# lorenzsp/EMRI_FrequencyDomainWaveforms

Hardware: AMD Instinct MI355X
Metric: FD waveforms/sec (2 yr, dt=10 s, ~3000 modes) at 1/2/4/8 GPUs; mode-sum HBM GB/s (higher is better)
Workload: dtype f64

## Files before the change

emri_frequencydomainwaveforms_amd/_lib.py:

```python

import ctypes
import os

_HERE = os.path.dirname(os.path.abspath(__file__))
LIB_PATH = os.environ.get("EFD_LIB") or os.path.join(_HERE, "libemrifd.so")

EFD_OK = 0
EFD_ERR_ARG = -1
EFD_ERR_HIP = -2
EFD_ERR_WORKSPACE = -3
EFD_CAUSTIC_SPA = 0
EFD_CAUSTIC_UNIFORM = 1
EFD_LOGLIKE_SCRATCH = 1024
EFD_INNER_SCRATCH = 2048
EFD_FISHER_MAX_PARAMS = 16
EFD_FISHER_SCRATCH = 139264
EFD_OVERLAP_MAX_ROWS = 64
EFD_OVERLAP_SCRATCH = 197632
EFD_BATCH_MAX = 16
EFD_HANN_ROWS_MAX = 16
EFD_HANN_LOCAL_PARTIALS = 4096
EFD_TD_SPLIT_SCRATCH = 1024
EFD_PAIR_MAX_ROWS = 64
EFD_PAIR_SCRATCH = 655360
EFD_DH_MAX_ROWS = 64
EFD_DH_SCRATCH = 196608
EFD_WINDOW_MAX_ROWS = 16
EFD_MODES_AMP_OVERFLOW = 1
EFD_TRAJ_MAX_LEN = 1024
EFD_NOISE_MAX_ROWS = 16
EFD_NOISE_DRAWS_PER_LAUNCH = 256
EFD_NOISE_SCRATCH = 1048576
EFD_TRAJ_OK = 0
EFD_TRAJ_BAD_SOURCE = 1
EFD_TRAJ_TOO_LONG = 2
EFD_TRAJ_STEP_FAILED = 3
EFD_TRAJ_STEP_CAP = 4
EFD_TRAJ_NO_BRACKET = 5

EXPORTED_SYMBOLS = (
    "efd_version",
    "efd_build_id",
# ... 35 lines not shown
    "efd_hann_loglike",
    "efd_hann_loglike_local",
    "efd_hann_loglike_local_partials",
    "efd_cosw_polarizations",
    "efd_cosw_loglike",
    "efd_loglike",
    "efd_inner_product",
    "efd_fisher_gram",
    "efd_overlap_rows",
    "efd_pair_stats",
    "efd_td_split_pair_stats",
    "efd_dh_hh_rows",
    "efd_window_rows",
    "efd_modesum_cpu",
    "efd_modesum_cpu_stats",
    "efd_spline_build_cpu",
    "efd_polarizations_cpu",
    "efd_loglike_cpu",
    "efd_inner_product_cpu",
    "efd_fisher_gram_cpu",
    "efd_overlap_rows_cpu",
    "efd_td_split_cpu",
    "efd_td_split_loglike_cpu",
    "efd_pair_stats_cpu",
    "efd_td_split_pair_stats_cpu",
    "efd_dh_hh_rows_cpu",
    "efd_window_rows_cpu",
    "efd_cpu_threads",
    "efd_cpu_last_error",
    "efd_host_trajectory",
# ... 286 lines not shown
    for name in ("efd_td_split_pair_stats", "efd_td_split_pair_stats_cpu"):
        getattr(lib, name).restype = ctypes.c_int
        getattr(lib, name).argtypes = [vp, i64, i64, i32, dbl, vp, i64, vp, vp, vp, vp, vp]
    for name in ("efd_dh_hh_rows", "efd_dh_hh_rows_cpu"):
        getattr(lib, name).restype = ctypes.c_int
        getattr(lib, name).argtypes = [vp, i64, i32, vp, vp, i32, i64, vp, vp, vp]
    for name in ("efd_window_rows", "efd_window_rows_cpu"):
        getattr(lib, name).restype = ctypes.c_int
        getattr(lib, name).argtypes = [vp, i64, ctypes.POINTER(vp), i32, vp, i64, vp]
    if hasattr(lib, "efd_modesum_cpu"):
        lib.efd_modesum_cpu.restype = ctypes.c_int
        lib.efd_modesum_cpu.argtypes = [ctypes.POINTER(ModesumArgs), vp, sz, vp]
        lib.efd_modesum_cpu_stats.restype = ctypes.c_int
        lib.efd_modesum_cpu_stats.argtypes = [ctypes.POINTER(i64), ctypes.POINTER(i64),
                                              ctypes.POINTER(i32)]
        lib.efd_spline_build_cpu.restype = ctypes.c_int
        lib.efd_spline_build_cpu.argtypes = [vp, ctypes.c_int, vp, ctypes.c_int, vp, vp]
        lib.efd_polarizations_cpu.restype = ctypes.c_int
        lib.efd_polarizations_cpu.argtypes = [vp, i64, i64, vp, vp, vp]
        lib.efd_loglike_cpu.restype = ctypes.c_int
        lib.efd_loglike_cpu.argtypes = [vp, vp, vp, i32, i64, vp, vp, vp]
        lib.efd_inner_product_cpu.restype = ctypes.c_int
        lib.efd_inner_product_cpu.argtypes = [vp, vp, vp, i32, i64, vp, vp, vp]
        lib.efd_fisher_gram_cpu.restype = ctypes.c_int
        lib.efd_fisher_gram_cpu.argtypes = [vp, i64, i32, i32, vp, vp, i64, vp, vp, vp, vp]
        lib.efd_cpu_threads.restype = ctypes.c_int
        lib.efd_cpu_threads.argtypes = [ctypes.c_int]
        lib.efd_cpu_last_error.restype = ctypes.c_int
        lib.efd_cpu_last_error.argtypes = [ctypes.c_char_p, ctypes.c_int]
    if hasattr(lib, "efd_host_trajectory"):
# ... 75 lines not shown
```

emri_frequencydomainwaveforms_amd/cputwin.py:

```python

import ctypes

import numpy as np

from . import _lib

CAUSTIC = {"spa": _lib.EFD_CAUSTIC_SPA, "uniform": _lib.EFD_CAUSTIC_UNIFORM}


def _lib_cpu():
    lib = _lib.load()
    if not hasattr(lib, "efd_modesum_cpu"):
        raise _lib.EFDError("libemrifd.so lacks efd_modesum_cpu: rebuild it")
    return lib


def set_threads(n):
    return int(_lib_cpu().efd_cpu_threads(int(n)))


def last_error():
    buf = ctypes.create_string_buffer(512)
    _lib_cpu().efd_cpu_last_error(buf, 512)
    return buf.value.decode(errors="replace")


def modesum(t, amp, phi_phi, phi_r, f_phi, f_r, m, n, ylm_p, ylm_m, freq, scale=1.0 + 0.0j,
            caustic="uniform", grid_symmetric=None, out=None, polarizations=False, k0=0,
            accumulate=False):
    lib = _lib_cpu()
    f64 = lambda x: np.ascontiguousarray(x, dtype=np.float64)
    c128 = lambda x: np.ascontiguousarray(x, dtype=np.complex128)
    i32 = lambda x: np.ascontiguousarray(x, dtype=np.int32)
    t, phi_phi, phi_r, f_phi, f_r, freq = (f64(x) for x in (t, phi_phi, phi_r, f_phi, f_r, freq))
    amp, ylm_p, ylm_m = c128(amp), c128(ylm_p), c128(ylm_m)
    m, n = i32(m), i32(n)
    nt, K = amp.shape
    nf = len(freq)
    if grid_symmetric is None:
        grid_symmetric = bool(np.array_equal(freq, -freq[::-1]))
    hp = hc = None
    new = np.zeros if accumulate else np.empty
    if polarizations:
        hp = new(nf - k0, dtype=np.complex128)
        hc = new(nf - k0, dtype=np.complex128)
        S = None
    else:
        S = out if out is not None else new(nf, dtype=np.complex128)
    p = lambda x: x.ctypes.data if x is not None else None
    sc = complex(scale)
    a = _lib.ModesumArgs(
        t=p(t), phi_phi=p(phi_phi), phi_r=p(phi_r), f_phi=p(f_phi), f_r=p(f_r), nt=nt,
        amp=p(amp), m=p(m), n=p(n), ylm_p=p(ylm_p), ylm_m=p(ylm_m), K=K, freq=p(freq), nf=nf,
        grid_symmetric=1 if grid_symmetric else 0, scale_re=sc.real, scale_im=sc.imag,
        caustic=CAUSTIC[caustic], accumulate=1 if accumulate else 0, out=p(S),
        prof_begin=None, prof_end=None, hp=p(hp), hc=p(hc), k0=int(k0))
    rc = lib.efd_modesum_cpu(ctypes.byref(a), None, 0, None)
    if rc != _lib.EFD_OK:
        raise _lib.EFDError(f"efd_modesum_cpu failed ({rc}): {last_error()}")
    return (hp, hc) if polarizations else S


def stats():
    c, e, g = ctypes.c_int64(0), ctypes.c_int64(0), ctypes.c_int32(0)
    _lib_cpu().efd_modesum_cpu_stats(ctypes.byref(c), ctypes.byref(e), ctypes.byref(g))
    return int(c.value), int(e.value), int(g.value)


def loglike(h, d, w):
    lib = _lib_cpu()
    h = np.ascontiguousarray(h, dtype=np.complex128)
    d = np.ascontiguousarray(d, dtype=np.complex128)
    w = np.ascontiguousarray(w, dtype=np.float64)
    if h.shape != d.shape or w.shape != d.shape or d.ndim != 2:
        raise ValueError("loglike: h, d, w must share one [nchan][nbin] shape")
# ... 7 lines not shown
```

emri_frequencydomainwaveforms_amd/csrc/emrifd.hip:

```cpp

#include "emrifd_layout.h"

#define EFD_VERSION 100

static thread_local std::string g_err;

int efdhip::fail(int code, const std::string& msg) {
    g_err = msg;
    return code;
}

namespace {

constexpr int NWAVE = TILE / 64;
constexpr int XCD_GROUP = 1024 / TILE;
constexpr int SEGWIN = TILE;
constexpr int PIECES = (int)sizeof(Item) / 16;
constexpr int B_PIECE = (int)offsetof(Item, b) / 16;
constexpr int ROUNDS = 2;
constexpr int NC = (ROUNDS * TILE) / PIECES;


__device__ __forceinline__ bool seg_hits_tile(int2 lh, int32_t tlo, int32_t thi) {
    return lh.y > tlo && lh.x < thi;
// ... 274 lines not shown
    r.shift = fdneg ? -192 : 192;
    r.kth = fdneg ? -KTH0 / VS : KTH0 / VS;
    return r;
}
__device__ __forceinline__ uint64_t class_mask(double x, int32_t cls) {
    uint64_t m;
    asm volatile("v_cmp_class_f64_e64 %0, %1, %2" : "=s"(m) : "v"(x), "s"(cls));
    return m;
}
__device__ __forceinline__ double ftz_select(bool ok, double v) {
    return __hiloint2double(ok ? __double2hiint(v) : 0, __double2loint(v));
}
constexpr int HDR_HB = TILE_LANES < 1024 ? 10 : 11;
constexpr uint32_t HDR_HM = (1u << HDR_HB) - 1u;
constexpr int HDR_S = 2 * HDR_HB, HDR_J = 2 * HDR_HB + 1, HDR_FD = 2 * HDR_HB + 4;
static_assert(FAST_J < 8, "header: jser in 3 bits");
static_assert(TILE_LANES < 2048 && HDR_FD + 2 <= 32, "header: one 32-bit word");
__device__ __forceinline__ uint32_t hdr_pack(uint32_t lo, uint32_t hi, int s, int32_t jser,
                                             int32_t fdneg) {
    return lo | (hi << HDR_HB) | ((uint32_t)s << HDR_S) | ((uint32_t)jser << HDR_J) |
           ((uint32_t)fdneg << HDR_FD);
}
__device__ __forceinline__ int32_t hdr_lo(uint32_t ha) { return (int32_t)(ha & HDR_HM); }
__device__ __forceinline__ int32_t hdr_hi(uint32_t ha) {
    return (int32_t)((ha >> HDR_HB) & HDR_HM);
}
__device__ __forceinline__ int hdr_s(uint32_t ha) { return (int)((ha >> HDR_S) & 1u); }
__device__ __forceinline__ uint32_t hdr_jser(uint32_t ha) { return (ha >> HDR_J) & 7u; }
__device__ __forceinline__ uint32_t hdr_fdneg(uint32_t ha) { return (ha >> HDR_FD) & 3u; }
__device__ __forceinline__ uint32_t hdr_safe(uint32_t ha) { return (ha >> (HDR_FD + 1)) & 1u; }
__device__ __forceinline__ bool hdr_test(uint32_t ha, uint32_t mask) {
    asm volatile("" : "+s"(ha));
    return (ha & mask) != 0;
}
__device__ __forceinline__ bool hdr_j3(uint32_t ha) {
    asm volatile("" : "+s"(ha));
    return hdr_jser(ha) >= 3u;
}
__device__ __forceinline__ bool hdr_j4(uint32_t ha) {
    asm volatile("" : "+s"(ha));
    return hdr_jser(ha) >= 4u;
}
__device__ __forceinline__ void spa_simple(const Item* __restrict__ it, double sfk, double stfk,
                                           const double2* __restrict__ sct, const RecSign& rs,
                                           double& wr, double& wi, double& w) {
    const double u = sfk - it->gx;
    const double tt = fma(fma(fma(it->ic[0], u, it->ic[1]), u, it->ic[2]), u, it->ic[3]);
    w = tt - it->tj;
    const double ph = fma(fma(fma(it->ph[0], w, it->ph[1]), w, it->ph[2]), w, it->ph[3]);
    const double fd = fma(fma(it->fd[0], w, it->fd[1]), w, it->fd[2]);
    const double amp = rsqrt_pos_sum(fabs(fd));
    const double psi0 = fma(stfk, tt, -ph);
    const double fdds = fma(fma(it->fdd[0], w, it->fdd[1]), w, it->fdd[2]);
    const double a3 = amp * amp * amp;
    const double t3 = fdds * a3;
    const double ww = t3 * t3;
// ... 13 lines not shown
    const double amp = rsqrt_pos_sum(fabs(fd));
    const double psi0 = fma(stfk, tt, -ph);
    const double fdds = fma(fma(it->fdd[0], w, it->fdd[1]), w, it->fdd[2]);
    const double a3 = amp * amp * amp;
    const double t3 = fdds * a3;
    const double ww = t3 * t3;
    const double uu = ww * ww;
    const double r = fma(45.7, uu * uu, 1.0 - uu);
    const double thn = ww * fma(-14.733333333333333333, uu, 1.0);
    const double am = amp * r;
    double sn, cs;
    sincos_tab(psi0, rs.shift, sct, sn, cs, thn, true, rs.kth, COS_A);
    wr = am * cs;
    wi = am * sn;
}
template <bool MASK, int NB>
__device__ __forceinline__ void env_record(const Item* __restrict__ it, const double* fk,
                                           const double* tfk, const double2* __restrict__ sct,
                                           const RecSign& rs, const uint64_t* am, double* wr,
                                           double* wi, double* w) {
    const double* e = env_of(it);
#pragma unroll
    for (int i = 0; i < NB; ++i) {
        const double u = fk[i] - it->gx;
        const double tt = fma(fma(fma(it->ic[0], u, it->ic[1]), u, it->ic[2]), u, it->ic[3]);
        w[i] = tt - it->tj;
        const double ph = fma(fma(fma(it->ph[0], w[i], it->ph[1]), w[i], it->ph[2]), w[i], it->ph[3]);
        const double psi0 = fma(tfk[i], tt, -ph);
        double amp = e[0];
#pragma unroll
        for (int c = 1; c <= ENV_DEG; ++c) amp = fma(amp, w[i], e[c]);
        if (MASK) amp = ftz_select(__builtin_amdgcn_inverse_ballot_w64(am[i]), amp);
        sincos_tab_amp(psi0, rs.shift, sct, amp, wr[i], wi[i]);
    }
}
template <int CAUSTIC>
__device__ __forceinline__ void spa_fast_m(const Item* __restrict__ it, double sfk, double stfk,
                                           uint32_t ha, uint64_t actm,
                                           const double2* __restrict__ sct,
                                           const RecSign& rs, double& wr, double& wi, double& w,
                                           uint64_t& needm) {
    const double u = sfk - it->gx;
    const double tt = fma(fma(fma(it->ic[0], u, it->ic[1]), u, it->ic[2]), u, it->ic[3]);
    w = tt - it->tj;
    const double ph = fma(fma(fma(it->ph[0], w, it->ph[1]), w, it->ph[2]), w, it->ph[3]);
    const double fd = fma(fma(it->fd[0], w, it->fd[1]), w, it->fd[2]);
    const double afd = fabs(fd);
    uint64_t goodm = ~0ull;
// ... 63 lines not shown
    exp_add(ay >= 153.0 ? 8 : ay >= 75.0 ? 9 : ay >= 48.0 ? 10 : ay >= 29.4 ? 11
            : ay >= 23.1 ? 12 : ay >= 20.3 ? 13 : ay >= 18.4 ? 14 : 15);
}
__device__ __forceinline__ void exp_chunk_balance(const int* wv) {
    int mx = 0, sm = 0;
    for (int w = 0; w < NWAVE; ++w) { mx = max(mx, wv[w]); sm += wv[w]; }
    exp_add(24, (unsigned long long)mx);
    exp_add(25, (unsigned long long)sm);
    exp_add(26);
}
__device__ __forceinline__ void exp_record(int64_t tile) {
    exp_add(0);
    if (tile < 16384) atomicAdd(&g_exp_tile[tile], 1u);
}
__device__ __forceinline__ void exp_record_class(uint32_t ha, bool partial) {
    exp_add(31 + min((int)hdr_jser(ha), 4));
    if (hdr_safe(ha)) exp_add(29);
    if (partial) exp_add(37);
    if (hdr_jser(ha) >= 3u) exp_add(38);
    if (!hdr_safe(ha)) exp_add(39);
}
template <int NB>
__device__ __forceinline__ void exp_cold(const bool (&need)[NB], int lane) {
    unsigned long long nl = 0;
#pragma unroll
    for (int i = 0; i < NB; ++i) nl += __popcll(__ballot(need[i]));
    if (lane == 0) {
        exp_add(16);
        exp_add(17, nl);
    }
}
__device__ __forceinline__ void exp_tile_clock(int64_t tile, unsigned long long t_start) {
    if (tile < 16384)
        g_exp_tclk[tile] = ((t_start & 0xffffffffull) << 32) |
// ... 308 lines not shown
        __syncthreads();

        for (int c = 0; c < nchunk; ++c) {
            tid = opq(tid0);
            lane = tid & 63;
            if (c + 1 < nchunk) EFD_GLDS(c + 1, (c + 1) & 1);
            const int nin = (int)rfl((uint32_t)min(NC, cnt - c * NC));
            const Item* stg = stage[c & 1];
            uint32_t hdr = 0;
            if (lane < nin) {
                const uint32_t kl = keys[c * NC + lane];
                const int sl = (int)(kl & 1);
                const Item* il = stg + lane;
                const uint32_t lo = (uint32_t)min(max(il->klo[sl] - tlo, 0), TILE_LANES);
                const uint32_t hi = (uint32_t)min(max(il->khi[sl] - tlo, 0), TILE_LANES);
                hdr = hdr_pack(lo, hi, sl, il->jser, il->fdneg);
            }
            EFD_EXP_DO(int nev = 0; if (c > 0 && tid == 0) exp_chunk_balance(wimb[(c - 1) & 1]);)
            for (int ii = 0; ii < nin; ++ii) {
                const uint32_t ha = (uint32_t)__builtin_amdgcn_readlane((int)hdr, ii);
                const int s = hdr_s(ha);
                const int32_t klo = tlo + hdr_lo(ha);
                const int32_t khi = tlo + hdr_hi(ha);
                const Item* it = stg + ii;
                if (khi <= e_lo || klo >= e_hi) {
                    EFD_EXP_DO(if (lane == 0) exp_add(3);)
                    continue;
                }
                EFD_EXP_DO(++nev; if (lane == 0) exp_record(tile);)
                bool anyneed = false;
                bool need[NB];
// ... 4 lines not shown
                        for (int i = 0; i < NB; ++i) {
                            fk[i] = -fk[i];
                            tfk[i] = -tfk[i];
                            own_i[i] = -own_i[i];
                            mir_i[i] = -mir_i[i];
                        }
                        s_cur = s;
                    }
                    const int J = CAUSTIC == EFD_CAUSTIC_UNIFORM ? (int)hdr_jser(ha) : FAST_J;
                    const double* xo = &it->b[0][0][0];
                    const double* xm = &it->b[1][0][0];
                    double wr[NB], wi[NB], w[NB];
                    uint64_t needm[NB], needany = 0;
                    const RecSign rs = rec_sign(hdr_fdneg(ha));
                    EFD_EXP_DO(if (lane == 0) exp_record_class(ha, e_lo < klo || khi < e_hi);)
                    if (CAUSTIC == EFD_CAUSTIC_UNIFORM && !hdr_test(ha, 7u << HDR_J)) {
                        if (!hdr_test((uint32_t)((e_lo - klo) | (khi - e_hi)) >> 31, 1u)) {
                            env_record<false, NB>(it, fk, tfk, sctab, rs, nullptr, wr, wi, w);
                        } else {
                            uint64_t am[NB];
#pragma unroll
                            for (int i = 0; i < NB; ++i) {
                                const int32_t base = e_lo + 64 * i;
                                am[i] = lane_range_mask(klo - base, khi - base);
                            }
                            env_record<true, NB>(it, fk, tfk, sctab, rs, am, wr, wi, w);
                        }
#pragma unroll
                        for (int i = 0; i < NB; ++i) need[i] = false;
                    } else
                    if (CAUSTIC == EFD_CAUSTIC_UNIFORM &&
                        !hdr_test(((uint32_t)((e_lo - klo) | (khi - e_hi)) >> 31) |
                                  ((hdr_jser(ha) + 5u) >> 3) |
                                  (hdr_safe(ha) ^ 1u), 1u)) {
#pragma unroll
                        for (int i = 0; i < NB; ++i) {
                            spa_simple(it, fk[i], tfk[i], sctab, rs, wr[i], wi[i], w[i]);
                            need[i] = false;
                        }
                    } else
                    if (CAUSTIC == EFD_CAUSTIC_UNIFORM &&
// ... 1404 lines not shown
```

emri_frequencydomainwaveforms_amd/csrc/emrifd_cpu.cpp:

```cpp
#include <algorithm>
#include <cmath>
#include <cstdint>
#include <cstdio>
#include <cstdlib>
#include <cstring>
#include <numeric>
#include <string>
#include <vector>

#include <omp.h>

#include "../../include/emrifd.h"
#include "emrifd_cpu_internal.h"

namespace efdcpu {

struct double2 {
    double x, y;
};
#define EFD_TABLE static const
#include "spa_tables.inc"
#undef EFD_TABLE

#include "emrifd_constants.h"
// ... 292 lines not shown
                    if (G0 != 0.0) {
                        const double xv = -(2.0 * G1) / (6.0 * G0);
                        if (xv > 0.0 && xv < dt) gmax = std::fmax(gmax, std::fabs(qv(3.0 * G0, 2.0 * G1, G2, xv)));
                    }
                    const double ymin = gmax > 0.0 ? TWO_PI * fdmin * fdmin * fdmin / (3.0 * gmax * gmax) / 1.1
                                                   : INFINITY;
                    int J = FAST_J;
                    for (int jj = 1; jj < FAST_J; ++jj)
                        if (ymin >= JSER_Y[jj]) { J = jj; break; }
                    it.jser = J;
                    it.envc = 0;
                    if (env_on && ymin >= ENV_MIN_Y) {
                        const double gq[3] = {3.0 * G0, 2.0 * G1, G2};
                        EnvFit E;
                        if (env_fit(it.fd, gq, it.dtj, (it.fdneg & 1) != 0, E)) {
                            it.envc = 1;
                            for (int c = 0; c <= ENV_DEG; ++c) it.env[c] = E.a[c];
                            for (int c = 0; c < 4; ++c) it.phE[c] = it.ph[c] - E.th[c];
                        }
                    }
                    const double Fj = knotF(a->f_phi, a->f_r, m, n, j);
                    const double Fj1 = knotF(a->f_phi, a->f_r, m, n, j + 1);
                    const double xlo = sg > 0 ? Fj : Fj1, xhi = sg > 0 ? Fj1 : Fj;
                    const bool strict = sg > 0 ? (j == ra) : (j + 1 == rb);
                    auto upper = [&](double v) { return (int64_t)(std::upper_bound(freq, freq + nf, v) - freq); };
                    auto lower = [&](double v) { return (int64_t)(std::lower_bound(freq, freq + nf, v) - freq); };
                    int64_t lo0 = upper(-xhi);
                    int64_t hi0 = strict ? lower(-xlo) : upper(-xlo);
                    int64_t lo1 = strict ? upper(xlo) : lower(xlo);
                    int64_t hi1 = lower(xhi);
                    auto clampr = [](int64_t& lo, int64_t& hi, int64_t lim) {
                        if (lo > lim) lo = lim;
// ... 200 lines not shown
        const int64_t qi = (int64_t)q;
        const int off = (int)((qi + shift) & 511);
        const double ts = T.s[off], tc = T.c[off];
        const double z = r * r;
        const double sr = std::fma(r * z, -1.6666666666666666e-01, r);
        const double cr = std::fma(z, COS_B, c0);
        const double sn = std::fma(ts, cr, tc * sr);
        const double cs = std::fma(tc, cr, -ts * sr);
        wr[i] = am * cs;
        wi[i] = am * sn;
        wv[i] = w;
        need[i] = !good;
    }
}

void spa_fast_env(const Rec& it, int s, const double* fk, int n, double* wr, double* wi,
                  double* wv, unsigned char* need) {
    const SinCosTable& T = sctab();
    const double sgn = s ? 1.0 : -1.0;
    const int shift = (it.fdneg & 1) ? -192 : 192;
    constexpr double INV_STEP = 81.48733086305042;
    constexpr double STEP_1 = 0.01227184630308513;
    constexpr double SHIFTER = 6755399441055744.0;
#pragma omp simd
    for (int i = 0; i < n; ++i) {
        const double g = sgn * fk[i];
        const double u = g - it.gx;
        const double tt = std::fma(std::fma(std::fma(it.ic[0], u, it.ic[1]), u, it.ic[2]), u, it.ic[3]);
        const double w = tt - it.tj;
        const bool good = (w >= 0.0) & (w < it.dtj);
        const double ph = std::fma(std::fma(std::fma(it.phE[0], w, it.phE[1]), w, it.phE[2]), w, it.phE[3]);
        const double psi0 = std::fma(TWO_PI * g, tt, -ph);
        double A = it.env[0];
        for (int c = 1; c <= ENV_DEG; ++c) A = std::fma(A, w, it.env[c]);
        const double am = good ? A : 0.0;
        const double qs = std::fma(psi0, INV_STEP, SHIFTER);
        const double q = qs - SHIFTER;
        const double r = std::fma(-q, STEP_1, psi0);
        const int64_t qi = (int64_t)q;
        const int off = (int)((qi + shift) & 511);
        const double ts = T.s[off], tc = T.c[off];
        const double z = r * r;
        const double sr = std::fma(r * z, -1.6666666666666666e-01, r);
        const double cr = std::fma(z, COS_B, COS_A);
        const double sn = std::fma(ts, cr, tc * sr);
        const double cs = std::fma(tc, cr, -ts * sr);
        wr[i] = am * cs;
        wi[i] = am * sn;
        wv[i] = w;
// ... 16 lines not shown
            for (int64_t t = it.klo[s] / TL; t <= (it.khi[s] - 1) / TL; ++t) ++cnt[t];
        }
    L.off.assign(ntiles + 1, 0);
    for (int64_t t = 0; t < ntiles; ++t) L.off[t + 1] = L.off[t] + cnt[t];
    L.ent.resize(L.off[ntiles]);
    std::vector<int64_t> pos(L.off.begin(), L.off.end() - 1);
    for (size_t r = 0; r < nrec; ++r)
        for (int s = 0; s < 2; ++s) {
            const Rec& it = P.recs[r];
            if (it.khi[s] <= it.klo[s]) continue;
            for (int64_t t = it.klo[s] / TL; t <= (it.khi[s] - 1) / TL; ++t)
                L.ent[pos[t]++] = (uint32_t)((r << 1) | (size_t)s);
        }
}

int modesum(const efd_modesum_args* a) {
    if (!a) return fail(EFD_ERR_ARG, "efd_modesum_cpu: NULL argument");
    if (!a->t || !a->phi_phi || !a->phi_r || !a->f_phi || !a->f_r || !a->amp || !a->m || !a->n ||
        !a->ylm_p || !a->ylm_m || !a->freq)
        return fail(EFD_ERR_ARG, "efd_modesum_cpu: NULL array");
    const bool pol = a->hp != nullptr || a->hc != nullptr;
    if (pol && (!a->hp || !a->hc || !a->grid_symmetric || a->k0 < 0 || a->k0 > a->nf))
        return fail(EFD_ERR_ARG, "efd_modesum_cpu: hp/hc need both pointers, a symmetric grid and 0 <= k0 <= nf");
    if (!a->out && !pol) return fail(EFD_ERR_ARG, "efd_modesum_cpu: no output (out or hp/hc)");
    if (a->nt < 2 || a->nt > MAX_NT) return fail(EFD_ERR_ARG, "efd_modesum_cpu: nt out of range");
    if (a->K <= 0 || a->K > MAX_K) return fail(EFD_ERR_ARG, "efd_modesum_cpu: K out of range [1, 8192]");
    if (a->nf <= 0 || a->nf >= (int64_t)INT32_MAX) return fail(EFD_ERR_ARG, "efd_modesum_cpu: nf out of range");
    if (a->caustic != EFD_CAUSTIC_SPA && a->caustic != EFD_CAUSTIC_UNIFORM)
        return fail(EFD_ERR_ARG, "efd_modesum_cpu: unknown caustic mode");
    for (int i = 1; i < a->nt; ++i)
        if (!(a->t[i] > a->t[i - 1])) return fail(EFD_ERR_ARG, "efd_modesum_cpu: t not increasing");
    const bool paired = a->grid_symmetric != 0;
    const int64_t nf = a->nf;
    const int64_t nl = paired ? (nf + 1) / 2 : nf;
    const int64_t nl1 = paired ? ((nf % 2) ? nl - 1 : nl) : nf;
    Prep P;
    const int rc = prepare(a, P, paired, nl, nl1);
    if (rc != EFD_OK) return rc;
    g_stats[0] = P.contributions;
    g_stats[1] = P.evaluations;
    g_stats[2] = P.G;
    const int64_t ntiles = (nl + TL - 1) / TL;
    TileLists L;
    build_tile_lists(P, ntiles, L);
    const double* freq = a->freq;
    const int caustic = a->caustic;
    const bool acc = a->accumulate != 0;
    const int64_t k0 = a->k0;
#pragma omp parallel num_threads(nthreads())
    {
        alignas(64) double fk[TL], own_r[TL], own_i[TL], mir_r[TL], mir_i[TL];
        alignas(64) double wr[TL], wi[TL], wv[TL];
// ... 4 lines not shown
            const int nln = (int)std::min<int64_t>(TL, nl - tlo);
            for (int i = 0; i < nln; ++i) fk[i] = freq[tlo + i];
            std::fill(own_r, own_r + TL, 0.0);
            std::fill(own_i, own_i + TL, 0.0);
            std::fill(mir_r, mir_r + TL, 0.0);
            std::fill(mir_i, mir_i + TL, 0.0);
            for (int64_t e = L.off[tile]; e < L.off[tile + 1]; ++e) {
                const uint32_t key = L.ent[e];
                const Rec& it = P.recs[key >> 1];
                const int s = (int)(key & 1u);
                const int lo = (int)std::max<int64_t>(it.klo[s] - tlo, 0);
                const int hi = (int)std::min<int64_t>(it.khi[s] - tlo, nln);
                if (hi <= lo) continue;
                const int n = hi - lo;
                if (caustic == EFD_CAUSTIC_UNIFORM) {
                    if (it.envc) spa_fast_env(it, s, fk + lo, n, wr, wi, wv, need);
                    else if (it.jser >= 3) spa_fast<EFD_CAUSTIC_UNIFORM, true>(it, s, fk + lo, n, wr, wi, wv, need);
                    else spa_fast<EFD_CAUSTIC_UNIFORM, false>(it, s, fk + lo, n, wr, wi, wv, need);
                } else {
                    spa_fast<EFD_CAUSTIC_SPA, false>(it, s, fk + lo, n, wr, wi, wv, need);
                }
                const double* X = &it.b[s][0][0];
                const double* Z = &it.b[1 - s][0][0];
                const double so = s ? -1.0 : 1.0;
#pragma omp simd
                for (int i = 0; i < n; ++i) {
                    const double w = wv[i];
                    const double xr = cubic(X, w), xi = cubic(X + 4, w);
                    const double zr = cubic(Z, w), zi = cubic(Z + 4, w);
                    const int k = lo + i;
                    own_r[k] = std::fma(-xi, wi[i], std::fma(xr, wr[i], own_r[k]));
// ... 68 lines not shown
    std::snprintf(buf, (size_t)len, "%s", efdcpu::g_err.c_str());
    return EFD_OK;
}

int efd_modesum_cpu(const efd_modesum_args* a, void* workspace, size_t workspace_bytes,
                    void* stream) {
    (void)workspace; (void)workspace_bytes; (void)stream;
    return efdcpu::modesum(a);
}

int efd_modesum_cpu_stats(int64_t* contributions, int64_t* evaluations, int32_t* groups) {
    if (contributions) *contributions = efdcpu::g_stats[0];
    if (evaluations) *evaluations = efdcpu::g_stats[1];
    if (groups) *groups = (int32_t)efdcpu::g_stats[2];
    return EFD_OK;
}

int efd_spline_build_cpu(const double* x, int n, const double* y, int ninterp, double* coef,
                         void* stream) {
    (void)stream;
    if (!x || !y || !coef || n < 2 || ninterp <= 0 || n > efdcpu::MAX_NT)
        return efdcpu::fail(EFD_ERR_ARG, "efd_spline_build_cpu: bad arguments");
    for (int i = 1; i < n; ++i)
        if (!(x[i] > x[i - 1])) return efdcpu::fail(EFD_ERR_ARG, "efd_spline_build_cpu: x not increasing");
#pragma omp parallel num_threads(efdcpu::nthreads())
    {
        std::vector<double> cp, dp, s, tq((size_t)(n - 1) * 4);
#pragma omp for schedule(static)
        for (int q = 0; q < ninterp; ++q) {
            efdcpu::spline_nak(n, [&](int i) { return x[i]; },
// ... 11 lines not shown
```

emri_frequencydomainwaveforms_amd/csrc/emrifd_prepare.hip:

```cpp

#include "emrifd_layout.h"

namespace {

constexpr int SPLINE_PF = 8;

__device__ __forceinline__ double spl_rcp(double x) {
#ifdef EFD_EXP_EXACT_RCP
    return 1.0 / x;
#endif
    double y = __builtin_amdgcn_rcp(x);
    double e = fma(-x, y, 1.0);
    y = fma(y, e, y);
    e = fma(-x, y, 1.0);
    return fma(y, e, y);
}

template <class FX, class FY, class FCP, class FDP, class FOUT>
__device__ void spline_not_a_knot(int n, FX X, FY Y, FCP CP, FDP DP, FOUT OUT) {
    if (n < 2) return;
    if (n == 2) {
        const double dx = X(1) - X(0);
        const double slope = (Y(1) - Y(0)) / dx;
        OUT(0, 0, 0.0); OUT(0, 1, 0.0); OUT(0, 2, slope); OUT(0, 3, Y(0));
// ... 1178 lines not shown
    if ((threadIdx.x & 63) == 0) {
        red[0][threadIdx.x >> 6] = contrib;
        red[1][threadIdx.x >> 6] = ev;
        red[2][threadIdx.x >> 6] = eev;
    }
    __syncthreads();
    if (threadIdx.x == 0) {
        const unsigned long long c = red[0][0] + red[0][1] + red[0][2] + red[0][3];
        const unsigned long long e = red[1][0] + red[1][1] + red[1][2] + red[1][3];
        const unsigned long long x = red[2][0] + red[2][1] + red[2][2] + red[2][3];
        if (c) atomicAdd((unsigned long long*)&hdr->contributions, c);
        if (e) atomicAdd((unsigned long long*)&hdr->evaluations, e);
        if (x) atomicAdd((unsigned long long*)&hdr->env_evaluations, x);
    }
}
__global__ __launch_bounds__(256) void k_items(const PrepBatch B) {
    const PrepView V(B);
    items_body(V.t, V.f_phi, V.f_r, V.gm, V.gn, V.gstart, V.nt, V.K, V.coefA, V.coefT, V.runs,
               V.freq, V.nf, V.paired, V.nl, V.nl1, V.items, V.ranges, V.header,
               (V.pcr & 1) != 0, V.env != 0);
}

__device__ __forceinline__ void slot_segment(const PrepView& V, int i,
                                             const int4* __restrict__ ranges, int G, int2& lh,
                                             int4& info) {
    const int h = i / (2 * MAXRUNS), r = (i >> 1) % MAXRUNS, sb = i & 1;
    const int ni = V.nt - 1;
    lh = make_int2(0, 0);
    info = make_int4(0, 0, 0, 0);
    const int32_t* rr = V.runs + (size_t)h * 4 * MAXRUNS + 4 * r;
    if (h < G && rr[2] != 0) {
// ... 508 lines not shown
```

emri_frequencydomainwaveforms_amd/csrc/env_fit.inc:

```

constexpr int ENV_DEG = 6;
constexpr double ENV_TOL_A = 1e-11;
constexpr double ENV_TOL_T = 1e-10;
constexpr double ENV_MIN_Y = 153.0;

struct EnvFit {
    double a[ENV_DEG + 1];
    double th[4];
};

EFD_HD inline void env_exact(const double* fd, const double* g, double thsign, double w, double& A,
                             double& th) {
    const double fdv = fma(fma(fd[0], w, fd[1]), w, fd[2]);
    const double fddv = fma(fma(g[0], w, g[1]), w, g[2]);
    const double r = env_rsqrt(fabs(fdv));
    const double r2 = r * r;
    const double wv = (3.0 / TWO_PI) * (fddv * fddv) * (r2 * r2 * r2);
    const double u = wv * wv;
    const double rho = fma(fma(fma(KRH[3], u, KRH[2]), u, KRH[1]), u, KRH[0]);
    const double thn = wv * fma(fma(fma(KTHN[3], u, KTHN[2]), u, KTHN[1]), u, KTHN[0]);
    A = rho * r;
    th = thsign * thn;
}

// ... 20 lines not shown
     -585.14285714285714286, 527.19549756118696301, -364.83060405905322015,
     130.20653506929482857}};
constexpr double ENV_W3[4][7] = {
    {-0.10165443621355265414, 0.10702091160166934744, 0.11930124891586627315,
     -0.14285714285714285714, -0.18986684997799971916, 0.30584819351622459786,
     0.90220807501493501199},
    {2.5185918758768087888, -2.2932605173801433673, -3.3408618646193829832,
     2.2857142857142857143, 6.1911009588307362656, 1.2760219621512775191,
     -6.6373067005735819373},
    {-8.6629029186417365166, 6.4590248426552300049, 11.945320391387904255,
     -2.2857142857142857143, -14.795559485599257537, -5.4417862874263641567,
     12.781617743338509665},
    {7.1481735539934153939, -3.9669370433605313872, -8.9136266256623872642, 0.0,
     8.9136266256623872642, 3.9669370433605313872, -7.1481735539934153939}};

template <int R>
EFD_HD inline void env_apply(const double (*M)[7], const double* f, double dtj, double* out) {
    const double r = 1.0 / dtj;
    double rk = 1.0;
#pragma unroll
    for (int i = 0; i < R; ++i) {
        double p = M[i][0] * f[0];
#pragma unroll
        for (int k = 1; k < 7; ++k) p = fma(M[i][k], f[k], p);
        out[R - 1 - i] = p * rk;
        rk *= r;
    }
}

EFD_HD inline bool env_fit(const double* fd, const double* g, double dtj, bool fdneg, EnvFit& E) {
    constexpr double X7[7] = {0.97492791218182360702, 0.78183148246802980871,
                              0.43388373911755812048, 0.0, -0.43388373911755812048,
                              -0.78183148246802980871, -0.97492791218182360702};
    constexpr double SC[8] = {0.0, 0.049515566048790436882, 0.18825509907063323474,
                              0.38873953302184279786, 0.61126046697815720214,
                              0.81174490092936676526, 0.95048443395120956312, 1.0};
    const double thsign = fdneg ? -KTH0 : KTH0;
    double fa[7], ft[7];
#pragma unroll
    for (int k = 0; k < 7; ++k) env_exact(fd, g, thsign, dtj * fma(0.5, X7[k], 0.5), fa[k], ft[k]);
    env_apply<ENV_DEG + 1>(ENV_W7, fa, dtj, E.a);
    env_apply<4>(ENV_W3, ft, dtj, E.th);
    double amax = 0.0, ea = 0.0, et = 0.0;
#pragma unroll
    for (int k = 0; k < 8; ++k) {
        const double w = dtj * SC[k];
        double A, th;
        env_exact(fd, g, thsign, w, A, th);
        double pa = E.a[0];
        for (int i = 1; i <= ENV_DEG; ++i) pa = fma(pa, w, E.a[i]);
        const double pt = fma(fma(fma(E.th[0], w, E.th[1]), w, E.th[2]), w, E.th[3]);
        amax = fmax(amax, fabs(A));
        ea = fmax(ea, fabs(pa - A));
        et = fmax(et, fabs(pt - th));
        if (!(fabs(A) < INFINITY && fabs(pa) < INFINITY && fabs(pt) < INFINITY)) return false;
    }
    return ea <= ENV_TOL_A * amax && et <= ENV_TOL_T;
}
```

include/emrifd.h:

```cpp
#ifndef EMRIFD_H
#define EMRIFD_H

#include <stddef.h>
#include <stdint.h>

#ifdef __cplusplus
extern "C" {
#endif

#define EFD_OK 0
#define EFD_ERR_ARG (-1)
#define EFD_ERR_HIP (-2)
#define EFD_ERR_WORKSPACE (-3)

#define EFD_CAUSTIC_SPA 0
#define EFD_CAUSTIC_UNIFORM 1

int efd_version(void);

const char* efd_build_id(void);

int efd_last_error(char* buf, int len);

int efd_spline_build(const double* x, int n, const double* y, int ninterp, double* coef,
// ... 176 lines not shown
                            const uint8_t* keep, double* out, double* scratch, void* stream);

#define EFD_DH_MAX_ROWS 64
#define EFD_DH_SCRATCH 196608
int efd_dh_hh_rows(const double* h, int64_t row_stride, int32_t nrow, const double* d,
                   const double* w, int32_t nchan, int64_t nbin, double* out, double* scratch,
                   void* stream);

#define EFD_WINDOW_MAX_ROWS 16
int efd_window_rows(const double* h, int64_t n, const double* const* win, int32_t nwin,
                    double* out, int64_t out_stride, void* stream);

int efd_modesum_cpu(const efd_modesum_args* a, void* workspace, size_t workspace_bytes,
                    void* stream);
int efd_modesum_cpu_stats(int64_t* contributions, int64_t* evaluations, int32_t* groups);
int efd_spline_build_cpu(const double* x, int n, const double* y, int ninterp, double* coef,
                         void* stream);
int efd_polarizations_cpu(const double* S, int64_t nf, int64_t k0, double* hp, double* hc,
                          void* stream);
int efd_loglike_cpu(const double* h, const double* d, const double* w, int32_t nchan,
                    int64_t nbin, double* out, double* scratch, void* stream);
int efd_inner_product_cpu(const double* a, const double* b, const double* w, int32_t nchan,
                          int64_t nbin, double* out, double* scratch, void* stream);
int efd_fisher_gram_cpu(const double* h, int64_t row_stride, int32_t nparam, int32_t npoint,
                        const double* coef, const double* w, int64_t nelem, double* dh,
                        double* gram, double* scratch, void* stream);
int efd_overlap_rows_cpu(const double* h, int64_t row_stride, int32_t nrow, const double* t,
                         const double* u, const double* w, int64_t nelem, double* out,
                         double* scratch, void* stream);
int efd_td_split_cpu(const double* Z, int64_t stride, int64_t n, int32_t rows, double gain,
// ... 146 lines not shown
```

Before: 1939.

## Economize envelope polynomial to degree 4 or 5 via Chebyshev truncation

After fitting the degree-6 amplitude envelope, the fit now tries to drop the top one or two coefficients using Chebyshev economization, and accepts the lower degree when the added error bound stays within the amplitude tolerance. The chosen degree is encoded in spare jser header codes, so the GPU mode-sum kernel dispatches to a templated envelope evaluator with fewer FMAs per frequency bin. The CPU twin is updated the same way and gains record and env-fit debug exports. The items prepare kernel also gets a launch-bounds occupancy hint. The cost is extra branching in the hot loop and slightly looser approximation error, still bounded by the tolerance.

```diff
diff --git a/emri_frequencydomainwaveforms_amd/_lib.py b/emri_frequencydomainwaveforms_amd/_lib.py
--- a/emri_frequencydomainwaveforms_amd/_lib.py
+++ b/emri_frequencydomainwaveforms_amd/_lib.py
@@ -26,6 +26,7 @@
 EFD_DH_MAX_ROWS = 64
 EFD_DH_SCRATCH = 196608
 EFD_WINDOW_MAX_ROWS = 16
+EFD_CPU_RECORD_COLS = 10
 EFD_MODES_AMP_OVERFLOW = 1
 EFD_TRAJ_MAX_LEN = 1024
 EFD_NOISE_MAX_ROWS = 16
@@ -91,6 +92,8 @@
     "efd_window_rows",
     "efd_modesum_cpu",
     "efd_modesum_cpu_stats",
+    "efd_modesum_cpu_records",
+    "efd_env_fit_cpu",
     "efd_spline_build_cpu",
     "efd_polarizations_cpu",
     "efd_loglike_cpu",
@@ -407,6 +410,11 @@
         lib.efd_modesum_cpu_stats.restype = ctypes.c_int
         lib.efd_modesum_cpu_stats.argtypes = [ctypes.POINTER(i64), ctypes.POINTER(i64),
                                               ctypes.POINTER(i32)]
+        lib.efd_modesum_cpu_records.restype = ctypes.c_int
+        lib.efd_modesum_cpu_records.argtypes = [ctypes.POINTER(ModesumArgs), vp, i64,
+                                                ctypes.POINTER(i64)]
+        lib.efd_env_fit_cpu.restype = ctypes.c_int
+        lib.efd_env_fit_cpu.argtypes = [vp, vp, dbl, i32, vp, vp]
         lib.efd_spline_build_cpu.restype = ctypes.c_int
         lib.efd_spline_build_cpu.argtypes = [vp, ctypes.c_int, vp, ctypes.c_int, vp, vp]
         lib.efd_polarizations_cpu.restype = ctypes.c_int
diff --git a/emri_frequencydomainwaveforms_amd/cputwin.py b/emri_frequencydomainwaveforms_amd/cputwin.py
--- a/emri_frequencydomainwaveforms_amd/cputwin.py
+++ b/emri_frequencydomainwaveforms_amd/cputwin.py
@@ -25,10 +25,8 @@
     return buf.value.decode(errors="replace")
 
 
-def modesum(t, amp, phi_phi, phi_r, f_phi, f_r, m, n, ylm_p, ylm_m, freq, scale=1.0 + 0.0j,
-            caustic="uniform", grid_symmetric=None, out=None, polarizations=False, k0=0,
-            accumulate=False):
-    lib = _lib_cpu()
+def _call_args(t, amp, phi_phi, phi_r, f_phi, f_r, m, n, ylm_p, ylm_m, freq, scale, caustic,
+               grid_symmetric):
     f64 = lambda x: np.ascontiguousarray(x, dtype=np.float64)
     c128 = lambda x: np.ascontiguousarray(x, dtype=np.complex128)
     i32 = lambda x: np.ascontiguousarray(x, dtype=np.int32)
@@ -36,9 +34,26 @@
     amp, ylm_p, ylm_m = c128(amp), c128(ylm_p), c128(ylm_m)
     m, n = i32(m), i32(n)
     nt, K = amp.shape
-    nf = len(freq)
     if grid_symmetric is None:
         grid_symmetric = bool(np.array_equal(freq, -freq[::-1]))
+    p = lambda x: x.ctypes.data
+    sc = complex(scale)
+    a = _lib.ModesumArgs(
+        t=p(t), phi_phi=p(phi_phi), phi_r=p(phi_r), f_phi=p(f_phi), f_r=p(f_r), nt=nt,
+        amp=p(amp), m=p(m), n=p(n), ylm_p=p(ylm_p), ylm_m=p(ylm_m), K=K, freq=p(freq),
+        nf=len(freq), grid_symmetric=1 if grid_symmetric else 0, scale_re=sc.real,
+        scale_im=sc.imag, caustic=CAUSTIC[caustic], accumulate=0, out=None, prof_begin=None,
+        prof_end=None, hp=None, hc=None, k0=0)
+    return a, (t, amp, phi_phi, phi_r, f_phi, f_r, m, n, ylm_p, ylm_m, freq)
+
+
+def modesum(t, amp, phi_phi, phi_r, f_phi, f_r, m, n, ylm_p, ylm_m, freq, scale=1.0 + 0.0j,
+            caustic="uniform", grid_symmetric=None, out=None, polarizations=False, k0=0,
+            accumulate=False):
+    lib = _lib_cpu()
+    a, keep = _call_args(t, amp, phi_phi, phi_r, f_phi, f_r, m, n, ylm_p, ylm_m, freq, scale,
+                         caustic, grid_symmetric)
+    nf = a.nf
     hp = hc = None
     new = np.zeros if accumulate else np.empty
     if polarizations:
@@ -48,17 +63,40 @@
     else:
         S = out if out is not None else new(nf, dtype=np.complex128)
     p = lambda x: x.ctypes.data if x is not None else None
-    sc = complex(scale)
-    a = _lib.ModesumArgs(
-        t=p(t), phi_phi=p(phi_phi), phi_r=p(phi_r), f_phi=p(f_phi), f_r=p(f_r), nt=nt,
-        amp=p(amp), m=p(m), n=p(n), ylm_p=p(ylm_p), ylm_m=p(ylm_m), K=K, freq=p(freq), nf=nf,
-        grid_symmetric=1 if grid_symmetric else 0, scale_re=sc.real, scale_im=sc.imag,
-        caustic=CAUSTIC[caustic], accumulate=1 if accumulate else 0, out=p(S),
-        prof_begin=None, prof_end=None, hp=p(hp), hc=p(hc), k0=int(k0))
+    a.accumulate, a.out, a.hp, a.hc, a.k0 = 1 if accumulate else 0, p(S), p(hp), p(hc), int(k0)
     rc = lib.efd_modesum_cpu(ctypes.byref(a), None, 0, None)
     if rc != _lib.EFD_OK:
         raise _lib.EFDError(f"efd_modesum_cpu failed ({rc}): {last_error()}")
     return (hp, hc) if polarizations else S
+
+
+RECORD_COLS = ("m", "n", "j", "klo0", "khi0", "klo1", "khi1", "env_degree", "jser", "evals")
+assert len(RECORD_COLS) == _lib.EFD_CPU_RECORD_COLS
+
+
+def records(t, amp, phi_phi, phi_r, f_phi, f_r, m, n, ylm_p, ylm_m, freq, scale=1.0 + 0.0j,
+            caustic="uniform", grid_symmetric=None):
+    lib = _lib_cpu()
+    a, keep = _call_args(t, amp, phi_phi, phi_r, f_phi, f_r, m, n, ylm_p, ylm_m, freq, scale,
+                         caustic, grid_symmetric)
+    cap = a.K * (a.nt - 1)
+    rows = np.zeros((cap, len(RECORD_COLS)), dtype=np.int64)
+    count = ctypes.c_int64(0)
+    rc = lib.efd_modesum_cpu_records(ctypes.byref(a), rows.ctypes.data, cap, ctypes.byref(count))
+    if rc != _lib.EFD_OK:
+        raise _lib.EFDError(f"efd_modesum_cpu_records failed ({rc}): {last_error()}")
+    return rows[:count.value]
+
+
+def env_fit(fd, g, dtj, fdneg):
+    fd = np.ascontiguousarray(fd, dtype=np.float64)
+    g = np.ascontiguousarray(g, dtype=np.float64)
+    if fd.shape != (3,) or g.shape != (3,):
+        raise ValueError("env_fit: fd and g are quadratics (3 coefficients)")
+    a, th = np.zeros(7), np.zeros(4)
+    deg = _lib_cpu().efd_env_fit_cpu(fd.ctypes.data, g.ctypes.data, float(dtj),
+                                     1 if fdneg else 0, a.ctypes.data, th.ctypes.data)
+    return int(deg), a, th
 
 
 def stats():
diff --git a/emri_frequencydomainwaveforms_amd/csrc/emrifd.hip b/emri_frequencydomainwaveforms_amd/csrc/emrifd.hip
--- a/emri_frequencydomainwaveforms_amd/csrc/emrifd.hip
+++ b/emri_frequencydomainwaveforms_amd/csrc/emrifd.hip
@@ -312,7 +312,9 @@
 constexpr int HDR_HB = TILE_LANES < 1024 ? 10 : 11;
 constexpr uint32_t HDR_HM = (1u << HDR_HB) - 1u;
 constexpr int HDR_S = 2 * HDR_HB, HDR_J = 2 * HDR_HB + 1, HDR_FD = 2 * HDR_HB + 4;
-static_assert(FAST_J < 8, "header: jser in 3 bits");
+constexpr uint32_t HDR_J_ENV5 = 5u, HDR_J_ENV4 = 6u;
+static_assert(FAST_J < HDR_J_ENV5 && HDR_J_ENV4 < 8, "header: jser and the envelope codes in 3 bits");
+static_assert(ENV_DEG == 6 && ENV_DEG_MIN == 4, "header: one code per envelope degree");
 static_assert(TILE_LANES < 2048 && HDR_FD + 2 <= 32, "header: one 32-bit word");
 __device__ __forceinline__ uint32_t hdr_pack(uint32_t lo, uint32_t hi, int s, int32_t jser,
                                              int32_t fdneg) {
@@ -338,6 +340,14 @@
 __device__ __forceinline__ bool hdr_j4(uint32_t ha) {
     asm volatile("" : "+s"(ha));
     return hdr_jser(ha) >= 4u;
+}
+__device__ __forceinline__ bool hdr_env(uint32_t ha) {
+    return !hdr_test(ha + (3u << HDR_J), 4u << HDR_J);
+}
+__device__ __forceinline__ int32_t hdr_j_of(const Item* it) {
+    if (it->jser != 0) return it->jser;
+    const int sk = env_skip(env_of(it));
+    return sk == 0 ? 0 : (sk == 1 ? (int32_t)HDR_J_ENV5 : (int32_t)HDR_J_ENV4);
 }
 __device__ __forceinline__ void spa_simple(const Item* __restrict__ it, double sfk, double stfk,
                                            const double2* __restrict__ sct, const RecSign& rs,
@@ -381,12 +391,13 @@
     wr = am * cs;
     wi = am * sn;
 }
-template <bool MASK, int NB>
+template <bool MASK, int NB, int DEG>
 __device__ __forceinline__ void env_record(const Item* __restrict__ it, const double* fk,
                                            const double* tfk, const double2* __restrict__ sct,
                                            const RecSign& rs, const uint64_t* am, double* wr,
                                            double* wi, double* w) {
-    const double* e = env_of(it);
+    static_assert(DEG >= ENV_DEG_MIN && DEG <= ENV_DEG, "envelope degree");
+    const double* e = env_of(it) + (ENV_DEG - DEG);
 #pragma unroll
     for (int i = 0; i < NB; ++i) {
         const double u = fk[i] - it->gx;
@@ -396,9 +407,26 @@
         const double psi0 = fma(tfk[i], tt, -ph);
         double amp = e[0];
 #pragma unroll
-        for (int c = 1; c <= ENV_DEG; ++c) amp = fma(amp, w[i], e[c]);
+        for (int c = 1; c <= DEG; ++c) amp = fma(amp, w[i], e[c]);
         if (MASK) amp = ftz_select(__builtin_amdgcn_inverse_ballot_w64(am[i]), amp);
         sincos_tab_amp(psi0, rs.shift, sct, amp, wr[i], wi[i]);
+    }
+}
+template <bool MASK, int NB>
+__device__ __forceinline__ void env_record_j(uint32_t ha, const Item* __restrict__ it,
+                                             const double* fk, const double* tfk,
+                                             const double2* __restrict__ sct, const RecSign& rs,
+                                             const uint64_t* am, double* wr, double* wi,
+                                             double* w) {
+    if (!hdr_test(ha, 7u << HDR_J)) {
+        asm volatile("");
+        env_record<MASK, NB, ENV_DEG>(it, fk, tfk, sct, rs, am, wr, wi, w);
+    } else if (hdr_test(ha, (HDR_J_ENV5 & ~HDR_J_ENV4) << HDR_J)) {
+        asm volatile("");
+        env_record<MASK, NB, 5>(it, fk, tfk, sct, rs, am, wr, wi, w);
+    } else {
+        asm volatile("");
+        env_record<MASK, NB, 4>(it, fk, tfk, sct, rs, am, wr, wi, w);
     }
 }
 template <int CAUSTIC>
@@ -492,10 +520,11 @@
     if (tile < 16384) atomicAdd(&g_exp_tile[tile], 1u);
 }
 __device__ __forceinline__ void exp_record_class(uint32_t ha, bool partial) {
-    exp_add(31 + min((int)hdr_jser(ha), 4));
+    const uint32_t j = hdr_jser(ha);
+    exp_add(j == HDR_J_ENV5 ? 30 : j == HDR_J_ENV4 ? 7 : 31 + min((int)j, 4));
     if (hdr_safe(ha)) exp_add(29);
     if (partial) exp_add(37);
-    if (hdr_jser(ha) >= 3u) exp_add(38);
+    if (j >= 3u && j <= (uint32_t)FAST_J) exp_add(38);
     if (!hdr_safe(ha)) exp_add(39);
 }
 template <int NB>
@@ -834,7 +863,7 @@
                 const Item* il = stg + lane;
                 const uint32_t lo = (uint32_t)min(max(il->klo[sl] - tlo, 0), TILE_LANES);
                 const uint32_t hi = (uint32_t)min(max(il->khi[sl] - tlo, 0), TILE_LANES);
-                hdr = hdr_pack(lo, hi, sl, il->jser, il->fdneg);
+                hdr = hdr_pack(lo, hi, sl, hdr_j_of(il), il->fdneg);
             }
             EFD_EXP_DO(int nev = 0; if (c > 0 && tid == 0) exp_chunk_balance(wimb[(c - 1) & 1]);)
             for (int ii = 0; ii < nin; ++ii) {
@@ -869,9 +898,9 @@
                     uint64_t needm[NB], needany = 0;
                     const RecSign rs = rec_sign(hdr_fdneg(ha));
                     EFD_EXP_DO(if (lane == 0) exp_record_class(ha, e_lo < klo || khi < e_hi);)
-                    if (CAUSTIC == EFD_CAUSTIC_UNIFORM && !hdr_test(ha, 7u << HDR_J)) {
+                    if (CAUSTIC == EFD_CAUSTIC_UNIFORM && hdr_env(ha)) {
                         if (!hdr_test((uint32_t)((e_lo - klo) | (khi - e_hi)) >> 31, 1u)) {
-                            env_record<false, NB>(it, fk, tfk, sctab, rs, nullptr, wr, wi, w);
+                            env_record_j<false, NB>(ha, it, fk, tfk, sctab, rs, nullptr, wr, wi, w);
                         } else {
                             uint64_t am[NB];
 #pragma unroll
@@ -879,7 +908,7 @@
                                 const int32_t base = e_lo + 64 * i;
                                 am[i] = lane_range_mask(klo - base, khi - base);
                             }
-                            env_record<true, NB>(it, fk, tfk, sctab, rs, am, wr, wi, w);
+                            env_record_j<true, NB>(ha, it, fk, tfk, sctab, rs, am, wr, wi, w);
                         }
 #pragma unroll
                         for (int i = 0; i < NB; ++i) need[i] = false;
diff --git a/emri_frequencydomainwaveforms_amd/csrc/emrifd_cpu.cpp b/emri_frequencydomainwaveforms_amd/csrc/emrifd_cpu.cpp
--- a/emri_frequencydomainwaveforms_amd/csrc/emrifd_cpu.cpp
+++ b/emri_frequencydomainwaveforms_amd/csrc/emrifd_cpu.cpp
@@ -330,8 +330,8 @@
                         const double gq[3] = {3.0 * G0, 2.0 * G1, G2};
                         EnvFit E;
                         if (env_fit(it.fd, gq, it.dtj, (it.fdneg & 1) != 0, E)) {
-                            it.envc = 1;
                             for (int c = 0; c <= ENV_DEG; ++c) it.env[c] = E.a[c];
+                            it.envc = ENV_DEG - env_skip(it.env);
                             for (int c = 0; c < 4; ++c) it.phE[c] = it.ph[c] - E.th[c];
                         }
                     }
@@ -562,6 +562,7 @@
     }
 }
 
+template <int DEG>
 void spa_fast_env(const Rec& it, int s, const double* fk, int n, double* wr, double* wi,
                   double* wv, unsigned char* need) {
     const SinCosTable& T = sctab();
@@ -579,8 +580,9 @@
         const bool good = (w >= 0.0) & (w < it.dtj);
         const double ph = std::fma(std::fma(std::fma(it.phE[0], w, it.phE[1]), w, it.phE[2]), w, it.phE[3]);
         const double psi0 = std::fma(TWO_PI * g, tt, -ph);
-        double A = it.env[0];
-        for (int c = 1; c <= ENV_DEG; ++c) A = std::fma(A, w, it.env[c]);
+        const double* e = it.env + (ENV_DEG - DEG);
+        double A = e[0];
+        for (int c = 1; c <= DEG; ++c) A = std::fma(A, w, e[c]);
         const double am = good ? A : 0.0;
         const double qs = std::fma(psi0, INV_STEP, SHIFTER);
         const double q = qs - SHIFTER;
@@ -627,15 +629,11 @@
         }
 }
 
-int modesum(const efd_modesum_args* a) {
+int check_inputs(const efd_modesum_args* a) {
     if (!a) return fail(EFD_ERR_ARG, "efd_modesum_cpu: NULL argument");
     if (!a->t || !a->phi_phi || !a->phi_r || !a->f_phi || !a->f_r || !a->amp || !a->m || !a->n ||
         !a->ylm_p || !a->ylm_m || !a->freq)
         return fail(EFD_ERR_ARG, "efd_modesum_cpu: NULL array");
-    const bool pol = a->hp != nullptr || a->hc != nullptr;
-    if (pol && (!a->hp || !a->hc || !a->grid_symmetric || a->k0 < 0 || a->k0 > a->nf))
-        return fail(EFD_ERR_ARG, "efd_modesum_cpu: hp/hc need both pointers, a symmetric grid and 0 <= k0 <= nf");
-    if (!a->out && !pol) return fail(EFD_ERR_ARG, "efd_modesum_cpu: no output (out or hp/hc)");
     if (a->nt < 2 || a->nt > MAX_NT) return fail(EFD_ERR_ARG, "efd_modesum_cpu: nt out of range");
     if (a->K <= 0 || a->K > MAX_K) return fail(EFD_ERR_ARG, "efd_modesum_cpu: K out of range [1, 8192]");
     if (a->nf <= 0 || a->nf >= (int64_t)INT32_MAX) return fail(EFD_ERR_ARG, "efd_modesum_cpu: nf out of range");
@@ -643,12 +641,55 @@
         return fail(EFD_ERR_ARG, "efd_modesum_cpu: unknown caustic mode");
     for (int i = 1; i < a->nt; ++i)
         if (!(a->t[i] > a->t[i - 1])) return fail(EFD_ERR_ARG, "efd_modesum_cpu: t not increasing");
-    const bool paired = a->grid_symmetric != 0;
+    return EFD_OK;
+}
+
+int prepare_call(const efd_modesum_args* a, Prep& P, bool& paired, int64_t& nl) {
+    paired = a->grid_symmetric != 0;
     const int64_t nf = a->nf;
-    const int64_t nl = paired ? (nf + 1) / 2 : nf;
+    nl = paired ? (nf + 1) / 2 : nf;
     const int64_t nl1 = paired ? ((nf % 2) ? nl - 1 : nl) : nf;
+    return prepare(a, P, paired, nl, nl1);
+}
+
+int records(const efd_modesum_args* a, int64_t* rows, int64_t capacity, int64_t* count) {
+    int rc = check_inputs(a);
+    if (rc != EFD_OK) return rc;
+    if (!count || capacity < 0 || (capacity > 0 && !rows))
+        return fail(EFD_ERR_ARG, "efd_modesum_cpu_records: bad output arguments");
     Prep P;
-    const int rc = prepare(a, P, paired, nl, nl1);
+    bool paired;
+    int64_t nl;
+    rc = prepare_call(a, P, paired, nl);
+    if (rc != EFD_OK) return rc;
+    const int ni = P.nt - 1;
+    const int64_t nrec = (int64_t)P.recs.size();
+    for (int64_t r = 0; r < std::min(nrec, capacity); ++r) {
+        const Rec& it = P.recs[(size_t)r];
+        const int g = (int)(r / ni);
+        const int64_t mult = paired && P.gm[g] != 0 ? 2 : 1;
+        int64_t* o = rows + r * EFD_CPU_RECORD_COLS;
+        o[0] = P.gm[g]; o[1] = P.gn[g]; o[2] = r - (int64_t)g * ni;
+        o[3] = it.klo[0]; o[4] = it.khi[0]; o[5] = it.klo[1]; o[6] = it.khi[1];
+        o[7] = it.envc; o[8] = it.jser;
+        o[9] = ((int64_t)(it.khi[0] - it.klo[0]) + (it.khi[1] - it.klo[1])) * mult;
+    }
+    *count = nrec;
+    return EFD_OK;
+}
+
+int modesum(const efd_modesum_args* a) {
+    int rc = check_inputs(a);
+    if (rc != EFD_OK) return rc;
+    const bool pol = a->hp != nullptr || a->hc != nullptr;
+    if (pol && (!a->hp || !a->hc || !a->grid_symmetric || a->k0 < 0 || a->k0 > a->nf))
+        return fail(EFD_ERR_ARG, "efd_modesum_cpu: hp/hc need both pointers, a symmetric grid and 0 <= k0 <= nf");
+    if (!a->out && !pol) return fail(EFD_ERR_ARG, "efd_modesum_cpu: no output (out or hp/hc)");
+    bool paired;
+    int64_t nl;
+    const int64_t nf = a->nf;
+    Prep P;
+    rc = prepare_call(a, P, paired, nl);
     if (rc != EFD_OK) return rc;
     g_stats[0] = P.contributions;
     g_stats[1] = P.evaluations;
@@ -683,7 +724,9 @@
                 if (hi <= lo) continue;
                 const int n = hi - lo;
                 if (caustic == EFD_CAUSTIC_UNIFORM) {
-                    if (it.envc) spa_fast_env(it, s, fk + lo, n, wr, wi, wv, need);
+                    if (it.envc == ENV_DEG) spa_fast_env<ENV_DEG>(it, s, fk + lo, n, wr, wi, wv, need);
+                    else if (it.envc == 5) spa_fast_env<5>(it, s, fk + lo, n, wr, wi, wv, need);
+                    else if (it.envc == 4) spa_fast_env<4>(it, s, fk + lo, n, wr, wi, wv, need);
                     else if (it.jser >= 3) spa_fast<EFD_CAUSTIC_UNIFORM, true>(it, s, fk + lo, n, wr, wi, wv, need);
                     else spa_fast<EFD_CAUSTIC_UNIFORM, false>(it, s, fk + lo, n, wr, wi, wv, need);
                 } else {
@@ -782,6 +825,23 @@
     if (evaluations) *evaluations = efdcpu::g_stats[1];
     if (groups) *groups = (int32_t)efdcpu::g_stats[2];
     return EFD_OK;
+}
+
+int efd_modesum_cpu_records(const efd_modesum_args* a, int64_t* rows, int64_t capacity,
+                            int64_t* count) {
+    return efdcpu::records(a, rows, capacity, count);
+}
+
+int efd_env_fit_cpu(const double* fd, const double* g, double dtj, int32_t fdneg, double* a,
+                    double* th) {
+    if (!fd || !g || !a || !th || !(dtj > 0.0))
+        return efdcpu::fail(0, "efd_env_fit_cpu: bad arguments");
+    efdcpu::EnvFit E;
+    const int deg = efdcpu::env_fit(fd, g, dtj, fdneg != 0, E);
+    if (deg == 0) return 0;
+    for (int c = 0; c <= efdcpu::ENV_DEG; ++c) a[c] = E.a[c];
+    for (int c = 0; c < 4; ++c) th[c] = E.th[c];
+    return efdcpu::ENV_DEG - efdcpu::env_skip(E.a);
 }
 
 int efd_spline_build_cpu(const double* x, int n, const double* y, int ninterp, double* coef,
diff --git a/emri_frequencydomainwaveforms_amd/csrc/emrifd_prepare.hip b/emri_frequencydomainwaveforms_amd/csrc/emrifd_prepare.hip
--- a/emri_frequencydomainwaveforms_amd/csrc/emrifd_prepare.hip
+++ b/emri_frequencydomainwaveforms_amd/csrc/emrifd_prepare.hip
@@ -1216,7 +1216,7 @@
         if (x) atomicAdd((unsigned long long*)&hdr->env_evaluations, x);
     }
 }
-__global__ __launch_bounds__(256) void k_items(const PrepBatch B) {
+__global__ __launch_bounds__(256, 4) void k_items(const PrepBatch B) {
     const PrepView V(B);
     items_body(V.t, V.f_phi, V.f_r, V.gm, V.gn, V.gstart, V.nt, V.K, V.coefA, V.coefT, V.runs,
                V.freq, V.nf, V.paired, V.nl, V.nl1, V.items, V.ranges, V.header,
diff --git a/emri_frequencydomainwaveforms_amd/csrc/env_fit.inc b/emri_frequencydomainwaveforms_amd/csrc/env_fit.inc
--- a/emri_frequencydomainwaveforms_amd/csrc/env_fit.inc
+++ b/emri_frequencydomainwaveforms_amd/csrc/env_fit.inc
@@ -1,5 +1,6 @@
 
 constexpr int ENV_DEG = 6;
+constexpr int ENV_DEG_MIN = 4;
 constexpr double ENV_TOL_A = 1e-11;
 constexpr double ENV_TOL_T = 1e-10;
 constexpr double ENV_MIN_Y = 153.0;
@@ -58,6 +59,9 @@
     {7.1481735539934153939, -3.9669370433605313872, -8.9136266256623872642, 0.0,
      8.9136266256623872642, 3.9669370433605313872, -7.1481735539934153939}};
 
+constexpr double ENV_T5[7] = {-1.0, 50.0, -400.0, 1120.0, -1280.0, 512.0, 0.0};
+constexpr double ENV_T6[7] = {1.0, -72.0, 840.0, -3584.0, 6912.0, -6144.0, 2048.0};
+
 template <int R>
 EFD_HD inline void env_apply(const double (*M)[7], const double* f, double dtj, double* out) {
     const double r = 1.0 / dtj;
@@ -72,7 +76,11 @@
     }
 }
 
-EFD_HD inline bool env_fit(const double* fd, const double* g, double dtj, bool fdneg, EnvFit& E) {
+EFD_HD inline int env_skip(const double* a) {
+    return a[0] != 0.0 ? 0 : (a[1] != 0.0 ? 1 : ENV_DEG - ENV_DEG_MIN);
+}
+
+EFD_HD inline int env_fit(const double* fd, const double* g, double dtj, bool fdneg, EnvFit& E) {
     constexpr double X7[7] = {0.97492791218182360702, 0.78183148246802980871,
                               0.43388373911755812048, 0.0, -0.43388373911755812048,
                               -0.78183148246802980871, -0.97492791218182360702};
@@ -97,7 +105,24 @@
         amax = fmax(amax, fabs(A));
         ea = fmax(ea, fabs(pa - A));
         et = fmax(et, fabs(pt - th));
-        if (!(fabs(A) < INFINITY && fabs(pa) < INFINITY && fabs(pt) < INFINITY)) return false;
+        if (!(fabs(A) < INFINITY && fabs(pa) < INFINITY && fabs(pt) < INFINITY)) return 0;
     }
-    return ea <= ENV_TOL_A * amax && et <= ENV_TOL_T;
+    const double tol = ENV_TOL_A * amax;
+    if (!(ea <= tol && et <= ENV_TOL_T)) return 0;
+    const double u6d = E.a[0] * dtj, v5 = fma(-ENV_T6[5] / ENV_T6[6], u6d, E.a[1]);
+    const double d2 = dtj * dtj, d5 = d2 * d2 * dtj;
+    const double b5 = fma(fabs(u6d * d5), 1.0 / ENV_T6[6], ea);
+    const double b4 = fma(fabs(v5 * d5), 1.0 / ENV_T5[5], b5);
+    if (!(b5 <= tol)) return ENV_DEG;
+    const int deg = b4 <= tol ? 4 : 5;
+    const double s5 = deg == 4 ? v5 : 0.0;
+    double q = dtj;
+#pragma unroll
+    for (int i = ENV_DEG - 2; i >= 0; --i) {
+        E.a[ENV_DEG - i] -= fma(u6d, ENV_T6[i] / ENV_T6[6], s5 * (ENV_T5[i] / ENV_T5[5])) * q;
+        q *= dtj;
+    }
+    E.a[1] = deg == 4 ? 0.0 : v5;
+    E.a[0] = 0.0;
+    return deg;
 }
diff --git a/include/emrifd.h b/include/emrifd.h
--- a/include/emrifd.h
+++ b/include/emrifd.h
@@ -214,6 +214,11 @@
 int efd_modesum_cpu(const efd_modesum_args* a, void* workspace, size_t workspace_bytes,
                     void* stream);
 int efd_modesum_cpu_stats(int64_t* contributions, int64_t* evaluations, int32_t* groups);
+#define EFD_CPU_RECORD_COLS 10
+int efd_modesum_cpu_records(const efd_modesum_args* a, int64_t* rows, int64_t capacity,
+                            int64_t* count);
+int efd_env_fit_cpu(const double* fd, const double* g, double dtj, int32_t fdneg, double* a,
+                    double* th);
 int efd_spline_build_cpu(const double* x, int n, const double* y, int ninterp, double* coef,
                          void* stream);
 int efd_polarizations_cpu(const double* S, int64_t nf, int64_t k0, double* hp, double* hc,
```

Result: no change. 1945 (median of 6 runs) (+0.3%).
